# 294coder/Dif-PAN

Hardware: AMD Instinct MI355X
Metric: fused megapixels/sec at T=1000, WV3 64x64x8 tiles (higher is better)
Workload: dtype f32-class (f16x2 split); 1 GPU; WV3 pansharpening, batch 64 of 64x64x8 tiles per GPU, T=1000 DDPM p_sample, fp32; tiles_per_gpu=64, tiles_total=64, T=1000, model_evaluations=1000, sampler=ddpm, parallelism=tile-shard x1, launches_per_denoising_step=132

## Files before the change

### dif-pan_amd/csrc/ddif_dev.h

```cpp
#pragma once
#include <hip/hip_runtime.h>

#ifdef DDIF_EMU
typedef hipemu_f32x16 f32x16;
typedef hipemu_f32x4 f32x4;
#define DDIF_MFMA_32x32x2(a, b, c) hipemu_mfma_32x32x2((a), (b), (c))
#define DDIF_MFMA_16x16x4(a, b, c) hipemu_mfma_16x16x4((a), (b), (c))
static inline f32x16 ddif_mfma_bf16_emu(float4 a, float4 b, f32x16 c) {
    hipemu_u32x4 ua, ub;
    __builtin_memcpy(&ua, &a, 16);
    __builtin_memcpy(&ub, &b, 16);
    return hipemu_mfma_32x32x16_bf16(ua, ub, c);
}
#define DDIF_MFMA_32x32x16_BF16(a, b, c) ddif_mfma_bf16_emu((a), (b), (c))
static inline f32x16 ddif_mfma_f16_emu(float4 a, float4 b, f32x16 c) {
    hipemu_u32x4 ua, ub;
    __builtin_memcpy(&ua, &a, 16);
    __builtin_memcpy(&ub, &b, 16);
    return hipemu_mfma_32x32x16_f16(ua, ub, c);
}
#define DDIF_MFMA_32x32x16_F16(a, b, c) ddif_mfma_f16_emu((a), (b), (c))
#define DDIF_DYN_SMEM(name) char* name = hipemu::tctx().dyn_smem
#define DDIF_SCHED_FENCE() ((void)0)
#else
typedef float f32x16 __attribute__((ext_vector_type(16)));
typedef float f32x4 __attribute__((ext_vector_type(4)));
#define DDIF_MFMA_32x32x2(a, b, c) __builtin_amdgcn_mfma_f32_32x32x2f32((a), (b), (c), 0, 0, 0)
#define DDIF_MFMA_16x16x4(a, b, c) __builtin_amdgcn_mfma_f32_16x16x4f32((a), (b), (c), 0, 0, 0)
typedef __bf16 ddif_bf16x8 __attribute__((ext_vector_type(8)));
#define DDIF_MFMA_32x32x16_BF16(a, b, c) \
    __builtin_amdgcn_mfma_f32_32x32x16_bf16(__builtin_bit_cast(ddif_bf16x8, (a)), __builtin_bit_cast(ddif_bf16x8, (b)), (c), 0, 0, 0)
typedef _Float16 ddif_f16x8 __attribute__((ext_vector_type(8)));
#define DDIF_MFMA_32x32x16_F16(a, b, c) \
    __builtin_amdgcn_mfma_f32_32x32x16_f16(__builtin_bit_cast(ddif_f16x8, (a)), __builtin_bit_cast(ddif_f16x8, (b)), (c), 0, 0, 0)
#define DDIF_DYN_SMEM(name) extern __shared__ __attribute__((aligned(16))) char name[]
#define DDIF_SCHED_FENCE() __builtin_amdgcn_sched_barrier(0)
#endif

#define DDIF_WAVE 64
#define DDIF_GN_EPS 1e-5

#ifdef DDIF_EMU
static inline long long wall_clock64() { return 0; }
#endif

namespace ddif {

__device__ __forceinline__ float dd_exp(float x) { return expf(x); }
__device__ __forceinline__ float dd_sigmoid(float x) {
#ifdef DDIF_EMU
    return 1.0f / (1.0f + exp2f(-1.4426950408889634f * x));
#else
    return __builtin_amdgcn_rcpf(1.0f + __builtin_amdgcn_exp2f(-1.4426950408889634f * x));
#endif
}
__device__ __forceinline__ float dd_silu(float x) { return x * dd_sigmoid(x); }
__device__ __forceinline__ float dd_exp2_fast(float x) {
#ifdef DDIF_EMU
    return exp2f(x);
#else
    return __builtin_amdgcn_exp2f(x);
#endif
}
__device__ __forceinline__ float dd_rcp_fast(float x) {
#ifdef DDIF_EMU
    return 1.0f / x;
#else
    return __builtin_amdgcn_rcpf(x);
#endif
}

__device__ __forceinline__ unsigned dd_bf16_bits(float x) {
    const unsigned u = __builtin_bit_cast(unsigned, x);
    return (u + 0x7fffu + ((u >> 16) & 1u)) >> 16;
}
__device__ __forceinline__ float dd_bf16_val(unsigned b) { return __builtin_bit_cast(float, b << 16); }
__device__ __forceinline__ void dd_split3(float x, unsigned* hi, unsigned* mid, unsigned* lo) {
    const unsigned h = dd_bf16_bits(x);
    const float r1 = x - dd_bf16_val(h);
    const unsigned m = dd_bf16_bits(r1);
    const float r2 = r1 - dd_bf16_val(m);
    *hi = h;
    *mid = m;
    *lo = dd_bf16_bits(r2);
}

__device__ __forceinline__ void dd_split3_pair(float a, float b, unsigned* hi, unsigned* mid, unsigned* lo) {
#ifdef DDIF_EMU
    unsigned ha, ma, la, hb, mb, lb;
    dd_split3(a, &ha, &ma, &la);
    dd_split3(b, &hb, &mb, &lb);
    *hi = ha | (hb << 16);
    *mid = ma | (mb << 16);
    *lo = la | (lb << 16);
#else
    typedef float v2f __attribute__((ext_vector_type(2)));
    typedef __bf16 v2b __attribute__((ext_vector_type(2)));
    const v2f v = {a, b};
    const unsigned H = __builtin_bit_cast(unsigned, __builtin_convertvector(v, v2b));
    const v2f r1 = {a - __builtin_bit_cast(float, H << 16), b - __builtin_bit_cast(float, H & 0xffff0000u)};
    const unsigned M = __builtin_bit_cast(unsigned, __builtin_convertvector(r1, v2b));
    const v2f r2 = {r1.x - __builtin_bit_cast(float, M << 16), r1.y - __builtin_bit_cast(float, M & 0xffff0000u)};
    *hi = H;
    *mid = M;
    *lo = __builtin_bit_cast(unsigned, __builtin_convertvector(r2, v2b));
#endif
}

__device__ __forceinline__ unsigned dd_bf16_pair(float a, float b) {
#ifdef DDIF_EMU
    return dd_bf16_bits(a) | (dd_bf16_bits(b) << 16);
#else
    typedef float v2f __attribute__((ext_vector_type(2)));
    typedef __bf16 v2b __attribute__((ext_vector_type(2)));
    const v2f v = {a, b};
    return __builtin_bit_cast(unsigned, __builtin_convertvector(v, v2b));
#endif
}

#define DDIF_F16_ASCALE 16.0f
#define DDIF_F16_WSCALE 1024.0f
#define DDIF_F16_OSCALE (1.0f / (DDIF_F16_ASCALE * DDIF_F16_WSCALE))
#define DDIF_F16_AMAX 4094.0f
#define DDIF_F16_WMAX 63.9f
#ifdef DDIF_EMU
static inline unsigned dd_f16_bits(float x) { return hipemu_f32_to_f16(x); }
static inline float dd_f16_val(unsigned b) { return hipemu_f16_to_f32((unsigned short)b); }
#endif
__device__ __forceinline__ void dd_split2_pair(float a, float b, unsigned* hi, unsigned* lo) {
#ifdef DDIF_EMU
    const unsigned ha = dd_f16_bits(a), hb = dd_f16_bits(b);
    *hi = ha | (hb << 16);
    *lo = dd_f16_bits(a - dd_f16_val(ha)) | (dd_f16_bits(b - dd_f16_val(hb)) << 16);
#else
    typedef float v2f __attribute__((ext_vector_type(2)));
    typedef _Float16 v2h __attribute__((ext_vector_type(2)));
    const v2f v = {a, b};
    const v2h H = __builtin_convertvector(v, v2h);
    const v2f r = {a - (float)H.x, b - (float)H.y};
    *hi = __builtin_bit_cast(unsigned, H);
    *lo = __builtin_bit_cast(unsigned, __builtin_convertvector(r, v2h));
#endif
}
__device__ __forceinline__ float dd_silu_scaled(float x, float inv_s) {
#ifdef DDIF_EMU
    return x * (1.0f / fmaf(exp2f(-1.4426950408889634f * x), inv_s, inv_s));
#else
    return x * __builtin_amdgcn_rcpf(fmaf(__builtin_amdgcn_exp2f(-1.4426950408889634f * x), inv_s, inv_s));
#endif
}

__device__ __forceinline__ int dd_late(int v) {
#if !defined(DDIF_EMU) && defined(__HIP_DEVICE_COMPILE__)
    asm volatile("" : "+v"(v));
#endif
    return v;
}

template <int BYTES>
__device__ __forceinline__ void dd_touch_kernargs() {
#if !defined(DDIF_EMU) && defined(__HIP_DEVICE_COMPILE__)
    const unsigned long long ka = (unsigned long long)__builtin_amdgcn_kernarg_segment_ptr();
    static_assert(BYTES >= 4 && BYTES <= 448, "kernarg touch: up to eight loads");
    constexpr int NL = (BYTES + 63) / 64 + 1;
#define DD_KA_OFF(i) ((i) * 64 < BYTES - 4 ? (i) * 64 : BYTES - 4)
    [[maybe_unused]] unsigned d0, d1, d2, d3, d4, d5, d6, d7;
    if constexpr (NL == 2) asm volatile("s_load_dword %0, %2, %3\n\ts_load_dword %1, %2, %4\n\ts_waitcnt lgkmcnt(0)" : "=&s"(d0), "=&s"(d1) : "s"(ka), "n"(DD_KA_OFF(0)), "n"(DD_KA_OFF(1)) : "memory");
    else if constexpr (NL == 3) asm volatile("s_load_dword %0, %3, %4\n\ts_load_dword %1, %3, %5\n\ts_load_dword %2, %3, %6\n\ts_waitcnt lgkmcnt(0)" : "=&s"(d0), "=&s"(d1), "=&s"(d2) : "s"(ka), "n"(DD_KA_OFF(0)), "n"(DD_KA_OFF(1)), "n"(DD_KA_OFF(2)) : "memory");
    else if constexpr (NL == 4) asm volatile("s_load_dword %0, %4, %5\n\ts_load_dword %1, %4, %6\n\ts_load_dword %2, %4, %7\n\ts_load_dword %3, %4, %8\n\ts_waitcnt lgkmcnt(0)" : "=&s"(d0), "=&s"(d1), "=&s"(d2), "=&s"(d3) : "s"(ka), "n"(DD_KA_OFF(0)), "n"(DD_KA_OFF(1)), "n"(DD_KA_OFF(2)), "n"(DD_KA_OFF(3)) : "memory");
    else if constexpr (NL == 5) asm volatile("s_load_dword %0, %5, %6\n\ts_load_dword %1, %5, %7\n\ts_load_dword %2, %5, %8\n\ts_load_dword %3, %5, %9\n\ts_load_dword %4, %5, %10\n\ts_waitcnt lgkmcnt(0)" : "=&s"(d0), "=&s"(d1), "=&s"(d2), "=&s"(d3), "=&s"(d4) : "s"(ka), "n"(DD_KA_OFF(0)), "n"(DD_KA_OFF(1)), "n"(DD_KA_OFF(2)), "n"(DD_KA_OFF(3)), "n"(DD_KA_OFF(4)) : "memory");
    else if constexpr (NL == 6) asm volatile("s_load_dword %0, %6, %7\n\ts_load_dword %1, %6, %8\n\ts_load_dword %2, %6, %9\n\ts_load_dword %3, %6, %10\n\ts_load_dword %4, %6, %11\n\ts_load_dword %5, %6, %12\n\ts_waitcnt lgkmcnt(0)" : "=&s"(d0), "=&s"(d1), "=&s"(d2), "=&s"(d3), "=&s"(d4), "=&s"(d5) : "s"(ka), "n"(DD_KA_OFF(0)), "n"(DD_KA_OFF(1)), "n"(DD_KA_OFF(2)), "n"(DD_KA_OFF(3)), "n"(DD_KA_OFF(4)), "n"(DD_KA_OFF(5)) : "memory");
    else if constexpr (NL == 7) asm volatile("s_load_dword %0, %7, %8\n\ts_load_dword %1, %7, %9\n\ts_load_dword %2, %7, %10\n\ts_load_dword %3, %7, %11\n\ts_load_dword %4, %7, %12\n\ts_load_dword %5, %7, %13\n\ts_load_dword %6, %7, %14\n\ts_waitcnt lgkmcnt(0)" : "=&s"(d0), "=&s"(d1), "=&s"(d2), "=&s"(d3), "=&s"(d4), "=&s"(d5), "=&s"(d6) : "s"(ka), "n"(DD_KA_OFF(0)), "n"(DD_KA_OFF(1)), "n"(DD_KA_OFF(2)), "n"(DD_KA_OFF(3)), "n"(DD_KA_OFF(4)), "n"(DD_KA_OFF(5)), "n"(DD_KA_OFF(6)) : "memory");
    else if constexpr (NL == 8) asm volatile("s_load_dword %0, %8, %9\n\ts_load_dword %1, %8, %10\n\ts_load_dword %2, %8, %11\n\ts_load_dword %3, %8, %12\n\ts_load_dword %4, %8, %13\n\ts_load_dword %5, %8, %14\n\ts_load_dword %6, %8, %15\n\ts_load_dword %7, %8, %16\n\ts_waitcnt lgkmcnt(0)" : "=&s"(d0), "=&s"(d1), "=&s"(d2), "=&s"(d3), "=&s"(d4), "=&s"(d5), "=&s"(d6), "=&s"(d7) : "s"(ka), "n"(DD_KA_OFF(0)), "n"(DD_KA_OFF(1)), "n"(DD_KA_OFF(2)), "n"(DD_KA_OFF(3)), "n"(DD_KA_OFF(4)), "n"(DD_KA_OFF(5)), "n"(DD_KA_OFF(6)), "n"(DD_KA_OFF(7)) : "memory");
#undef DD_KA_OFF
#endif
}

__device__ __forceinline__ void wg_work_range(int nwork, int* w0, int* w1, int xcd = 0) {
    const unsigned g = gridDim.x, n = (unsigned)nwork;
    const unsigned b = (xcd && (g & 7u) == 0u) ? (blockIdx.x & 7u) * (g >> 3) + (blockIdx.x >> 3) : blockIdx.x;
    const unsigned q = n / g, r = n - q * g;
    *w0 = (int)(b * q + (b * r) / g);
    *w1 = (int)((b + 1) * q + ((b + 1) * r) / g);
}

__device__ __forceinline__ float wave_sum(float v) {
#pragma unroll
    for (int m = 32; m >= 1; m >>= 1) v += __shfl_xor(v, m);
    return v;
}
__device__ __forceinline__ float wave_sum_fast(float v) {
#ifdef DDIF_EMU
#pragma unroll
    for (int m = 32; m >= 1; m >>= 1) v += __shfl_xor(v, m);
    return v;
#else
    v += __builtin_bit_cast(float, __builtin_amdgcn_update_dpp(0, __builtin_bit_cast(int, v), 0xB1, 0xf, 0xf, false));
    v += __builtin_bit_cast(float, __builtin_amdgcn_update_dpp(0, __builtin_bit_cast(int, v), 0x4E, 0xf, 0xf, false));
    v += __builtin_bit_cast(float, __builtin_amdgcn_update_dpp(0, __builtin_bit_cast(int, v), 0x124, 0xf, 0xf, false));
    v += __builtin_bit_cast(float, __builtin_amdgcn_update_dpp(0, __builtin_bit_cast(int, v), 0x128, 0xf, 0xf, false));
    v += __builtin_bit_cast(float, __builtin_amdgcn_update_dpp(0, __builtin_bit_cast(int, v), 0x142, 0xa, 0xf, false));
    v += __builtin_bit_cast(float, __builtin_amdgcn_update_dpp(0, __builtin_bit_cast(int, v), 0x143, 0xc, 0xf, false));
    return v;
#endif
}
__device__ __forceinline__ double wave_sum(double v) {
#pragma unroll
    for (int m = 32; m >= 1; m >>= 1) v += __shfl_xor(v, m);
    return v;
}
__device__ __forceinline__ double wave_sum_fast_f64(double v) {
#ifdef DDIF_EMU
    return wave_sum(v);
#else
#define DDIF_DPP_ADD_F64(ctrl, rmask)                                                                              \
    {                                                                                                              \
        const unsigned long long u = __builtin_bit_cast(unsigned long long, v);                                    \
        const int lo = __builtin_amdgcn_update_dpp(0, (int)(unsigned)u, ctrl, rmask, 0xf, false);                   \
        const int hi = __builtin_amdgcn_update_dpp(0, (int)(unsigned)(u >> 32), ctrl, rmask, 0xf, false);           \
        v += __builtin_bit_cast(double, ((unsigned long long)(unsigned)hi << 32) | (unsigned long long)(unsigned)lo); \
    }
    DDIF_DPP_ADD_F64(0xB1, 0xf)
    DDIF_DPP_ADD_F64(0x4E, 0xf)
    DDIF_DPP_ADD_F64(0x124, 0xf)
    DDIF_DPP_ADD_F64(0x128, 0xf)
    DDIF_DPP_ADD_F64(0x142, 0xa)
    DDIF_DPP_ADD_F64(0x143, 0xc)
#undef DDIF_DPP_ADD_F64
    const unsigned long long u = __builtin_bit_cast(unsigned long long, v);
    const unsigned lo = (unsigned)__builtin_amdgcn_readlane((int)(unsigned)u, 63), hi = (unsigned)__builtin_amdgcn_readlane((int)(unsigned)(u >> 32), 63);
    return __builtin_bit_cast(double, ((unsigned long long)hi << 32) | lo);
#endif
}
__device__ __forceinline__ float wave_max(float v) {
#pragma unroll
    for (int m = 32; m >= 1; m >>= 1) v = fmaxf(v, __shfl_xor(v, m));
    return v;
}

struct GnRedRec { const double* cpart; float* dgamma; float* dbeta; int C, nchunk, blk0, pad; };
struct GnPartials {
    double v[2][4][2];
};
__device__ __forceinline__ void gn_load_partials(const double* st0, int np0, const double* st1, int np1, int b, GnPartials* p) {
    const int lane = threadIdx.x & 63;
#pragma unroll
    for (int k = 0; k < 4; ++k) {
        const int i = lane + 64 * k;
        const int i0 = i < np0 ? i : np0 - 1;
        p->v[0][k][0] = st0[((size_t)b * np0 + i0) * 2 + 0];
        p->v[0][k][1] = st0[((size_t)b * np0 + i0) * 2 + 1];
        if (st1 != nullptr) {
            const int i1 = i < np1 ? i : np1 - 1;
            p->v[1][k][0] = st1[((size_t)b * np1 + i1) * 2 + 0];
            p->v[1][k][1] = st1[((size_t)b * np1 + i1) * 2 + 1];
        }
    }
}
__device__ __forceinline__ void gn_reduce_partials(const GnPartials& p, const double* st0, int np0, const double* st1, int np1, int b,
                                                    double count, float* mean_out, float* rstd_out) {
    const int lane = threadIdx.x & 63;
    double s = 0.0, ss = 0.0;
#pragma unroll
    for (int k = 0; k < 4; ++k)
        if (lane + 64 * k < np0) {
            s += p.v[0][k][0];
            ss += p.v[0][k][1];
        }
    for (int i = lane + 256; i < np0; i += 64) {
        s += st0[((size_t)b * np0 + i) * 2 + 0];
        ss += st0[((size_t)b * np0 + i) * 2 + 1];
    }
    if (st1 != nullptr) {
#pragma unroll
        for (int k = 0; k < 4; ++k)
            if (lane + 64 * k < np1) {
                s += p.v[1][k][0];
                ss += p.v[1][k][1];
            }
        for (int i = lane + 256; i < np1; i += 64) {
            s += st1[((size_t)b * np1 + i) * 2 + 0];
            ss += st1[((size_t)b * np1 + i) * 2 + 1];
        }
    }
    s = wave_sum_fast_f64(s);
    ss = wave_sum_fast_f64(ss);
    const double mean = s / count;
    double var = ss / count - mean * mean;
    if (var < 0.0) var = 0.0;
    *mean_out = (float)mean;
    *rstd_out = (float)(1.0 / sqrt(var + DDIF_GN_EPS));
}
__device__ __forceinline__ void gn_finalize_wave(const double* st0, int np0, const double* st1, int np1, int b,
                                                  double count, float* mean_out, float* rstd_out) {
    GnPartials p;
    gn_load_partials(st0, np0, st1, np1, b, &p);
    gn_reduce_partials(p, st0, np0, st1, np1, b, count, mean_out, rstd_out);
}

}
```

### dif-pan_amd/csrc/kernels_lr.h

```cpp
#pragma once
#include "kernels_conv.h"

namespace ddif {

#ifndef LR_ROWPAD
#define LR_ROWPAD 1
#endif
#if defined(DDIF_EMU) || !defined(__HIP_DEVICE_COMPILE__)
#define LR_PREFETCH_FENCE() ((void)0)
#elif defined(LR_NO_FENCE)
#define LR_PREFETCH_FENCE() ((void)0)
#else
#define LR_PREFETCH_FENCE() asm volatile("" ::: "memory")
#endif
template <int KS, int MB, int PRO, bool TALL = false, bool F16 = false, bool B1 = false>
struct LrGeom {
    static constexpr int NPL = F16 ? 2 : (B1 ? 1 : 3);
    static constexpr int TH = (TALL && MB == 4) ? 16 : 8, TW = (MB == 2 || TALL) ? 8 : 16;
    static constexpr int PAD = KS / 2;
    static constexpr int IH = TH + 2 * PAD, IW = TW + 2 * PAD;
    static constexpr int PC = (MB == 4 && KS == 3) ? 64 : 128;
    static constexpr int SP = PC / 16;
    static constexpr int APIX = SP * NPL * 8 + 4;
    static constexpr int RSL = (IW * APIX / 4) % 16;
    static constexpr int RPAD = LR_ROWPAD ? (((TW == 8 ? 8 : 0) - RSL + 16) % 16) * 4 : 0;
    static constexpr int AROW = IW * APIX + RPAD;
    static constexpr int AFL = IH * AROW;
    static constexpr int RFL = 4 * MB * 4 * 64 * 4;
    static constexpr size_t smem = (size_t)((AFL > RFL ? AFL : RFL) + 16) * sizeof(float);
    static constexpr int SPW = SP / 4;
    static constexpr int TAPS = KS * KS;
    static constexpr int U = KS == 3 ? TAPS : SPW;
};

template <int KS, int MB, int PRO, int EPI, int ABL = 0, bool F16 = false, bool B1 = false, bool ROWS = false>
__global__ __launch_bounds__(256) void conv_lr_kernel(ConvArgs a) {
    constexpr bool COLST = (EPI & EPI_COLST) != 0;
    static_assert(!COLST || KS == 1, "column statistics epilogue: 1x1 convs");
    static_assert(!F16 || PRO != PRO_COLSM, "f16x2: the column-softmax prologue stays on bf16x3");
    static_assert(!(F16 && B1), "one operand format");
    using G = LrGeom<KS, MB, PRO, COLST, F16, B1>;
    constexpr int NPL = G::NPL, SLF = NPL * 8;
    constexpr int WSTEP = NPL * 1024;
    constexpr int TH = G::TH, TW = G::TW, LP = G::PAD, LH = G::IH, LW = G::IW, IW = G::IW, PC = G::PC, SP = G::SP;
    constexpr int APIX = G::APIX, AROW = G::AROW, TAPS = G::TAPS, U = G::U, SPW = G::SPW;
    constexpr bool GNP = (PRO == PRO_GN || PRO == PRO_GN_SILU);
    static_assert(PRO == PRO_NONE || PRO == PRO_GN || PRO == PRO_GN_SILU || PRO == PRO_COLSM, "prologues of the low-resolution kernel");
    constexpr bool FILM = (EPI & EPI_FILM) != 0, RES = (EPI & EPI_RES) != 0, SILU = (EPI & EPI_SILU) != 0;
    constexpr int C4 = PC / 4;
    constexpr int PSTEP = 256 / C4;
    constexpr int NIT = ROWS ? LH : (LH * LW + PSTEP - 1) / PSTEP;
    static_assert(256 % C4 == 0, "staging geometry");
    static_assert(!ROWS || (KS == 3 && PSTEP == TW && PRO != PRO_COLSM), "row staging: 3x3 convs, one pass of the threads = one image row");

    dd_touch_kernargs<sizeof(ConvArgs)>();
    DDIF_DYN_SMEM(smem);
    float* As = reinterpret_cast<float*>(smem);
    float* Red = As;
    float* Sst = As + (G::AFL > G::RFL ? G::AFL : G::RFL);

    const int tid = threadIdx.x, lane = tid & 63;
#ifdef DDIF_EMU
    const int wave = tid >> 6;
#else
    const int wave = __builtin_amdgcn_readfirstlane(tid >> 6);
#endif
    const int h = lane >> 5, j = lane & 31;
    const int tiles = a.tiles_x * a.tiles_y;
    const int nwork = a.B * tiles * a.n_ct;
    int w0, w1;
    wg_work_range(nwork, &w0, &w1, a.xcd);
    const int Ctot = a.c0 + a.c1;
#ifdef DDIF_EMU
    const int ac0 = a.c0, ac1 = a.c1;
#else
    const int ac0 = __builtin_amdgcn_readfirstlane(a.c0), ac1 = __builtin_amdgcn_readfirstlane(a.c1);
#endif
    const int NS = (Ctot + 15) / 16;
    const int NSW = a.n_chunks * (KS == 3 ? 1 : 2);
    const int NP = (NS + SP - 1) / SP;
    const int c4 = tid % C4, p0 = tid / C4;
    const int stepv = a.step_ptr ? *a.step_ptr : 0;

    int abase[MB];
#pragma unroll
    for (int mb = 0; mb < MB; ++mb) {
        const int m = mb * 32 + j;
        abase[mb] = (m / TW) * AROW + (m % TW) * APIX + 4 * h;
    }

    int gn_b = -1;
    float mean = 0.f, rstd = 1.f;
    constexpr bool RANGE = F16 && !GNP && PRO != PRO_COLSM;
    [[maybe_unused]] float r_max = 0.f;

    for (int work = w0; work < w1; ++work) {
        const int pt = work / a.n_ct, ct = work - pt * a.n_ct;
        const int bl = pt / tiles, t = pt - bl * tiles;
        const int b = a.b0 + bl;
        const int oy0 = (t / a.tiles_x) * TH, ox0 = (t % a.tiles_x) * TW;

        [[maybe_unused]] GnPartials gp;
        const bool new_b = GNP && b != gn_b;
        if (new_b) gn_load_partials(a.st0, a.np0, a.st1, a.np1, b, &gp);

        const int co = ct * 32 + 8 * wave + 4 * h;
        const bool cok_o = co < a.Cout;
        const int coc = cok_o ? co : 0;
        const float4 bq = *reinterpret_cast<const float4*>(a.bias + coc);
        [[maybe_unused]] float4 e_res[RES ? MB : 1], e_fs[FILM ? MB : 1], e_fh[FILM ? MB : 1];
        bool pok[MB];
        size_t opix[MB];
#pragma unroll
        for (int mb = 0; mb < MB; ++mb) {
            const int m = mb * 32 + j;
            const int oy = oy0 + m / TW, ox = ox0 + m % TW;
            pok[mb] = (oy < a.Hout) & (ox < a.Wout) & cok_o;
            opix[mb] = pok[mb] ? ((size_t)b * a.Hout + oy) * a.Wout + ox : 0;
            if constexpr (RES) e_res[mb] = *reinterpret_cast<const float4*>(a.res + opix[mb] * a.Cout + coc);
            if constexpr (FILM) {
                e_fs[mb] = *reinterpret_cast<const float4*>(a.film + opix[mb] * 2 * a.Cout + coc);
                e_fh[mb] = *reinterpret_cast<const float4*>(a.film + opix[mb] * 2 * a.Cout + a.Cout + coc);
            }
        }

        const char* wbase = reinterpret_cast<const char*>(a.w + (size_t)b * a.w_bstride) + ((size_t)ct * NSW * TAPS) * WSTEP + (size_t)lane * 16;
        int pf_slab = wave, pf_tap = 0;
        float4 wr[U][NPL];
        auto ring_load = [&](int slot) {
            const int s = pf_slab < NS ? pf_slab : 0;
            const char* p = wbase + ((size_t)s * TAPS + pf_tap) * WSTEP;
#pragma unroll
            for (int q = 0; q < NPL; ++q) {
                if (ABL & 1) wr[slot][q] = make_float4(1e-3f * (float)q, 2e-3f, 3e-3f, 4e-3f);
                else wr[slot][q] = *reinterpret_cast<const float4*>(p + q * 1024);
            }
            if (++pf_tap == TAPS) {
                pf_tap = 0;
                pf_slab += 4;
            }
        };
#pragma unroll
        for (int u = 0; u < U; ++u) ring_load(u);

        float4 sv[NIT];
        [[maybe_unused]] float4 mxv[PRO == PRO_COLSM ? NIT : 1], smv[PRO == PRO_COLSM ? NIT : 1];
        [[maybe_unused]] float4 gq4, bq4;
        unsigned okm = 0;
        auto stage_load = [&](int ph) {
            const int c = ph * PC + c4 * 4;
            const bool cok = c < Ctot;
            const bool s0 = !cok || c < a.c0;
            const float* src = s0 ? a.in0 + (cok ? c : 0) : a.in1 + (c - a.c0);
            const int cs = s0 ? ac0 : ac1;
            okm = 0;
            if constexpr (ROWS) {
                const float* rp = src + (((size_t)b * a.Hin + oy0) * a.Win + p0) * cs;
                const ptrdiff_t rs = (ptrdiff_t)a.Win * cs;
#pragma unroll
                for (int it = 0; it < NIT; ++it) {
                    const int iy = oy0 - LP + it;
                    if ((iy >= 0) & (iy < a.Hin)) {
                        okm |= 1u << it;
                        if (ABL & 4) sv[it] = make_float4(0.5f, 0.25f, -0.5f, 0.125f);
                        else sv[it] = *reinterpret_cast<const float4*>(rp + (ptrdiff_t)(it - LP) * rs);
                    }
                }
            } else {
#pragma unroll
            for (int it = 0; it < NIT; ++it) {
                const int pix = p0 + it * PSTEP;
                const int py = pix / LW, px = pix - py * LW;
                const int iy = oy0 - LP + py, ix = ox0 - LP + px;
                const bool ok = (pix < LH * LW) & (iy >= 0) & (iy < a.Hin) & (ix >= 0) & (ix < a.Win) & cok;
                okm |= (ok ? 1u : 0u) << it;
                const int iyc = iy < 0 ? 0 : (iy >= a.Hin ? a.Hin - 1 : iy), ixc = ix < 0 ? 0 : (ix >= a.Win ? a.Win - 1 : ix);
                const size_t sp = ((size_t)b * a.Hin + iyc) * a.Win + ixc;
                if (ABL & 4) sv[it] = make_float4(0.5f, 0.25f, -0.5f, 0.125f);
                else sv[it] = *reinterpret_cast<const float4*>(src + sp * cs);
                if constexpr (PRO == PRO_COLSM) {
                    const size_t so = ((size_t)b * a.Win + ixc) * a.c0 + ((s0 && cok) ? c : 0);
                    mxv[it] = *reinterpret_cast<const float4*>(a.cs_mx + so);
                    smv[it] = *reinterpret_cast<const float4*>(a.cs_sm + so);
                }
            }
            }
            if constexpr (GNP) {
                gq4 = *reinterpret_cast<const float4*>(a.gamma + (cok ? c : 0));
                bq4 = *reinterpret_cast<const float4*>(a.beta + (cok ? c : 0));
            }
        };
        auto stage_write = [&](int ph) {
            const int c = ph * PC + c4 * 4;
            const bool cok = c < Ctot;
            const bool colsm = (PRO == PRO_COLSM) && cok && c < a.c0;
            const int slab_l = (c4 * 4) / 16, cin_slab = (c4 * 4) % 16;
            float ga[4] = {1.f, 1.f, 1.f, 1.f}, gb[4] = {0.f, 0.f, 0.f, 0.f};
            if constexpr (GNP) {
#pragma unroll
                for (int i = 0; i < 4; ++i) {
                    ga[i] = (&gq4.x)[i] * rstd;
                    gb[i] = (&bq4.x)[i] - mean * ga[i];
                    if constexpr (F16 && PRO == PRO_GN) {
                        ga[i] *= DDIF_F16_ASCALE;
                        gb[i] *= DDIF_F16_ASCALE;
                    }
                }
            }
#pragma unroll
            for (int it = 0; it < NIT; ++it) {
                const int pix = ROWS ? it * LW + p0 + LP : p0 + it * PSTEP;
                if constexpr (ROWS) {
                    if (!((okm >> it) & 1u)) {
                        float* d = &As[it * AROW + (p0 + LP) * APIX + slab_l * SLF + cin_slab / 2];
#pragma unroll
                        for (int q = 0; q < NPL; ++q) *reinterpret_cast<uint2*>(d + 8 * q) = make_uint2(0u, 0u);
                        continue;
                    }
                }
                const bool ok = ROWS ? cok : (okm >> it) & 1u;
                float v[4];
#pragma unroll
                for (int i = 0; i < 4; ++i) {
                    float x = (&sv[it].x)[i];
                    if constexpr (GNP) {
                        x = fmaf(x, ga[i], gb[i]);
                        if constexpr (PRO == PRO_GN_SILU) x = F16 ? dd_silu_scaled(x, 1.0f / DDIF_F16_ASCALE) : dd_silu(x);
                    } else if constexpr (F16) {
                        x *= DDIF_F16_ASCALE;
                    }
                    if constexpr (PRO == PRO_COLSM) {
                        if (colsm) x = dd_exp2_fast((x - (&mxv[it].x)[i]) * 1.4426950408889634f) * dd_rcp_fast((&smv[it].x)[i]);
                    }
                    v[i] = ok ? x : 0.f;
                }
                if constexpr (RANGE) r_max = fmaxf(fmaxf(r_max, fmaxf(fabsf(v[0]), fabsf(v[1]))), fmaxf(fabsf(v[2]), fabsf(v[3])));
                if (ROWS || pix < LH * LW) {
                    float* d = ROWS ? &As[it * AROW + (p0 + LP) * APIX + slab_l * SLF + cin_slab / 2] : &As[(pix / LW) * AROW + (pix % LW) * APIX + slab_l * SLF + cin_slab / 2];
                    if constexpr (B1) {
                        *reinterpret_cast<uint2*>(d) = make_uint2(dd_bf16_pair(v[0], v[1]), dd_bf16_pair(v[2], v[3]));
                    } else if constexpr (F16) {
                        unsigned h01, l01, h23, l23;
                        dd_split2_pair(v[0], v[1], &h01, &l01);
                        dd_split2_pair(v[2], v[3], &h23, &l23);
                        *reinterpret_cast<uint2*>(d) = make_uint2(h01, h23);
                        *reinterpret_cast<uint2*>(d + 8) = make_uint2(l01, l23);
                    } else {
                        unsigned h01, m01, l01, h23, m23, l23;
                        dd_split3_pair(v[0], v[1], &h01, &m01, &l01);
                        dd_split3_pair(v[2], v[3], &h23, &m23, &l23);
                        *reinterpret_cast<uint2*>(d) = make_uint2(h01, h23);
                        *reinterpret_cast<uint2*>(d + 8) = make_uint2(m01, m23);
                        *reinterpret_cast<uint2*>(d + 16) = make_uint2(l01, l23);
                    }
                }
            }
        };
        stage_load(0);
        if constexpr (ROWS) {
            constexpr int Q = (APIX - 4) / 4;
            for (int i = tid; i < LH * 2 * Q; i += 256) {
                const int r = i / (2 * Q), e = i - r * (2 * Q);
                *reinterpret_cast<float4*>(&As[r * AROW + (e >= Q ? (LW - 1) * APIX + (e - Q) * 4 : e * 4)]) = make_float4(0.f, 0.f, 0.f, 0.f);
            }
        }
        const float4 tq = *reinterpret_cast<const float4*>(a.tbias + (size_t)dd_late(stepv) * a.tb_rowstride + (size_t)b * a.tbias_stride + coc);

        if (new_b) {
            gn_reduce_partials(gp, a.st0, a.np0, a.st1, a.np1, b, (double)Ctot * a.Hin * a.Win, &mean, &rstd);
            gn_b = b;
        }
        f32x16 acc[MB];
#pragma unroll
        for (int mb = 0; mb < MB; ++mb)
#pragma unroll
            for (int r = 0; r < 16; ++r) acc[mb][r] = 0.f;

        for (int ph = 0; ph < NP; ++ph) {
            if (ph > 0) __syncthreads();
            stage_write(ph);
            if (ph + 1 < NP) stage_load(ph + 1);
            __syncthreads();
            const int s_end = (ph + 1) * SP < NS ? (ph + 1) * SP : NS;
            float4 xa[2][MB][NPL];
            auto a_load = [&](int buf, int sl, int tap) {
                const int aoff = (tap / KS) * AROW + (tap % KS) * APIX + sl * SLF;
#pragma unroll
                for (int q = 0; q < NPL; ++q)
#pragma unroll
                    for (int mb = 0; mb < MB; ++mb) xa[buf][mb][q] = *reinterpret_cast<const float4*>(&As[abase[mb] + aoff + q * 8]);
            };
#pragma unroll
            for (int k = 0; k < SPW; ++k) {
                const int sl = wave + 4 * k;
                if (ph * SP + sl < s_end) {
                    a_load(0, sl, 0);
#pragma unroll
                    for (int tap = 0; tap < TAPS; ++tap) {
                        constexpr int UU = U;
                        const int u = (k * TAPS + tap) % UU;
                        const int cur = tap & 1;
                        if (tap + 1 < TAPS) a_load(cur ^ 1, sl, tap + 1);
                        LR_PREFETCH_FENCE();
                        if (ABL & 2) {
#pragma unroll
                            for (int mb = 0; mb < MB; ++mb) acc[mb][0] += wr[u][0].x * xa[cur][mb][0].x + wr[u][NPL / 2].y * xa[cur][mb][NPL / 2].y + wr[u][NPL - 1].z * xa[cur][mb][NPL - 1].z;
                        } else if constexpr (B1) {
#pragma unroll
                            for (int mb = 0; mb < MB; ++mb) acc[mb] = DDIF_MFMA_32x32x16_BF16(wr[u][0], xa[cur][mb][0], acc[mb]);
                        } else if constexpr (F16) {
#pragma unroll
                            for (int mb = 0; mb < MB; ++mb) acc[mb] = DDIF_MFMA_32x32x16_F16(wr[u][NPL - 1], xa[cur][mb][0], acc[mb]);
#pragma unroll
                            for (int mb = 0; mb < MB; ++mb) acc[mb] = DDIF_MFMA_32x32x16_F16(wr[u][0], xa[cur][mb][NPL - 1], acc[mb]);
#pragma unroll
                            for (int mb = 0; mb < MB; ++mb) acc[mb] = DDIF_MFMA_32x32x16_F16(wr[u][0], xa[cur][mb][0], acc[mb]);
                        } else if constexpr (NPL == 3) {
#pragma unroll
                            for (int mb = 0; mb < MB; ++mb) acc[mb] = DDIF_MFMA_32x32x16_BF16(wr[u][2], xa[cur][mb][0], acc[mb]);
#pragma unroll
                            for (int mb = 0; mb < MB; ++mb) acc[mb] = DDIF_MFMA_32x32x16_BF16(wr[u][0], xa[cur][mb][2], acc[mb]);
#pragma unroll
                            for (int mb = 0; mb < MB; ++mb) acc[mb] = DDIF_MFMA_32x32x16_BF16(wr[u][1], xa[cur][mb][1], acc[mb]);
#pragma unroll
                            for (int mb = 0; mb < MB; ++mb) acc[mb] = DDIF_MFMA_32x32x16_BF16(wr[u][1], xa[cur][mb][0], acc[mb]);
#pragma unroll
                            for (int mb = 0; mb < MB; ++mb) acc[mb] = DDIF_MFMA_32x32x16_BF16(wr[u][0], xa[cur][mb][1], acc[mb]);
#pragma unroll
                            for (int mb = 0; mb < MB; ++mb) acc[mb] = DDIF_MFMA_32x32x16_BF16(wr[u][0], xa[cur][mb][0], acc[mb]);
                        }
                        if (pf_slab < NS) ring_load(u);
                    }
                }
            }
        }
        __syncthreads();
#pragma unroll
        for (int mb = 0; mb < MB; ++mb)
#pragma unroll
            for (int g = 0; g < 4; ++g)
                *reinterpret_cast<float4*>(&Red[(((wave * MB + mb) * 4 + g) * 64 + lane) * 4]) =
                    make_float4(acc[mb][4 * g + 0], acc[mb][4 * g + 1], acc[mb][4 * g + 2], acc[mb][4 * g + 3]);
        __syncthreads();
        float s1 = 0.f, s2 = 0.f;
        [[maybe_unused]] float colv[COLST ? MB : 1][4];
#pragma unroll
        for (int mb = 0; mb < MB; ++mb) {
            float4 pp[4];
#pragma unroll
            for (int w = 0; w < 4; ++w) pp[w] = *reinterpret_cast<const float4*>(&Red[(((w * MB + mb) * 4 + wave) * 64 + lane) * 4]);
            float v[4];
#pragma unroll
            for (int i = 0; i < 4; ++i) {
                float x = ((&pp[0].x)[i] + (&pp[1].x)[i]) + ((&pp[2].x)[i] + (&pp[3].x)[i]);
                x = F16 ? fmaf(x, DDIF_F16_OSCALE, (&bq.x)[i] + (&tq.x)[i]) : x + ((&bq.x)[i] + (&tq.x)[i]);
                if constexpr (FILM) x = x * (1.f + (&e_fs[mb].x)[i]) + (&e_fh[mb].x)[i];
                if constexpr (SILU) x = dd_silu(x);
                if constexpr (RES) x += (&e_res[mb].x)[i];
                v[i] = x;
            }
            if constexpr (COLST) {
#pragma unroll
                for (int i = 0; i < 4; ++i) colv[mb][i] = pok[mb] ? v[i] : -INFINITY;
            }
            if (pok[mb]) {
                if (!(ABL & 8) || v[0] == 12345.678f) *reinterpret_cast<float4*>(a.out + opix[mb] * a.Cout + co) = make_float4(v[0], v[1], v[2], v[3]);
                s1 += (v[0] + v[1]) + (v[2] + v[3]);
                s2 += (v[0] * v[0] + v[1] * v[1]) + (v[2] * v[2] + v[3] * v[3]);
            }
        }
        if constexpr (COLST) {
            float cm[4], cs[4];
#pragma unroll
            for (int i = 0; i < 4; ++i) {
                float m = colv[0][i];
#pragma unroll
                for (int mb = 1; mb < MB; ++mb) m = fmaxf(m, colv[mb][i]);
                m = fmaxf(m, __shfl_xor(m, 8));
                m = fmaxf(m, __shfl_xor(m, 16));
                float e = 0.f;
#pragma unroll
                for (int mb = 0; mb < MB; ++mb) e += dd_exp(colv[mb][i] - m);
                e += __shfl_xor(e, 8);
                e += __shfl_xor(e, 16);
                cm[i] = m;
                cs[i] = e;
            }
            const int ox = ox0 + (j & 7);
            if (j < 8 && ox < a.Wout && cok_o) {
                const size_t so = ((size_t)b * a.Wout + ox) * a.Cout + co;
                *reinterpret_cast<float4*>(a.cso_mx + so) = make_float4(cm[0], cm[1], cm[2], cm[3]);
                *reinterpret_cast<float4*>(a.cso_sm + so) = make_float4(cs[0], cs[1], cs[2], cs[3]);
            }
        }
        if (a.st_out) {
            const float t1 = wave_sum_fast(s1), t2 = wave_sum_fast(s2);
            if (lane == 63) {
                Sst[wave * 2 + 0] = t1;
                Sst[wave * 2 + 1] = t2;
            }
        }
        __syncthreads();
        if (a.st_out && tid == 0) {
            const size_t pi = ((size_t)b * (tiles * a.n_ct) + (size_t)t * a.n_ct + ct) * 2;
            a.st_out[pi + 0] = ((double)Sst[0] + (double)Sst[2]) + ((double)Sst[4] + (double)Sst[6]);
            a.st_out[pi + 1] = ((double)Sst[1] + (double)Sst[3]) + ((double)Sst[5] + (double)Sst[7]);
        }
    }
    if constexpr (RANGE) {
        if (a.range_flag && !(r_max < 65520.f)) *a.range_flag = 1;
    }
}

}
```

Before: 0.07849 MP/s.

## Cut address arithmetic and register pressure in LR conv kernel

```diff
diff --git a/dif-pan_amd/csrc/ddif_dev.h b/dif-pan_amd/csrc/ddif_dev.h
--- a/dif-pan_amd/csrc/ddif_dev.h
+++ b/dif-pan_amd/csrc/ddif_dev.h
@@ -291,6 +291,51 @@
     *mean_out = (float)mean;
     *rstd_out = (float)(1.0 / sqrt(var + DDIF_GN_EPS));
 }
+#ifndef DDIF_GN_SMALL_NP
+#define DDIF_GN_SMALL_NP 64
+#endif
+static_assert(DDIF_GN_SMALL_NP == 64 || DDIF_GN_SMALL_NP == 0, "one pair per lane is fetched ahead, or none is used");
+__device__ __forceinline__ void gn_load_partials_few(const double* st0, int np0, const double* st1, int np1, int b, GnPartials* p) {
+    const int lane = threadIdx.x & 63;
+    const unsigned i0 = (unsigned)(b * np0 + (lane < np0 ? lane : np0 - 1)) * 2u;
+    p->v[0][0][0] = st0[i0 + 0];
+    p->v[0][0][1] = st0[i0 + 1];
+    if (st1 != nullptr) {
+        const unsigned i1 = (unsigned)(b * np1 + (lane < np1 ? lane : np1 - 1)) * 2u;
+        p->v[1][0][0] = st1[i1 + 0];
+        p->v[1][0][1] = st1[i1 + 1];
+    }
+}
+__device__ __forceinline__ void gn_reduce_partials_few(const GnPartials& p, const double* st0, int np0, const double* st1, int np1, int b,
+                                                        double count, float* mean_out, float* rstd_out) {
+    const int lane = threadIdx.x & 63;
+    double s = 0.0, ss = 0.0;
+    if (DDIF_GN_SMALL_NP > 0 && lane < np0) {
+        s += p.v[0][0][0];
+        ss += p.v[0][0][1];
+    }
+    for (int i = lane + DDIF_GN_SMALL_NP; i < np0; i += 64) {
+        s += st0[((size_t)b * np0 + i) * 2 + 0];
+        ss += st0[((size_t)b * np0 + i) * 2 + 1];
+    }
+    if (st1 != nullptr) {
+        if (DDIF_GN_SMALL_NP > 0 && lane < np1) {
+            s += p.v[1][0][0];
+            ss += p.v[1][0][1];
+        }
+        for (int i = lane + DDIF_GN_SMALL_NP; i < np1; i += 64) {
+            s += st1[((size_t)b * np1 + i) * 2 + 0];
+            ss += st1[((size_t)b * np1 + i) * 2 + 1];
+        }
+    }
+    s = wave_sum_fast_f64(s);
+    ss = wave_sum_fast_f64(ss);
+    const double mean = s / count;
+    double var = ss / count - mean * mean;
+    if (var < 0.0) var = 0.0;
+    *mean_out = (float)mean;
+    *rstd_out = (float)(1.0 / sqrt(var + DDIF_GN_EPS));
+}
 __device__ __forceinline__ void gn_finalize_wave(const double* st0, int np0, const double* st1, int np1, int b,
                                                   double count, float* mean_out, float* rstd_out) {
     GnPartials p;
diff --git a/dif-pan_amd/csrc/kernels_lr.h b/dif-pan_amd/csrc/kernels_lr.h
--- a/dif-pan_amd/csrc/kernels_lr.h
+++ b/dif-pan_amd/csrc/kernels_lr.h
@@ -82,27 +82,27 @@
     const int c4 = tid % C4, p0 = tid / C4;
     const int stepv = a.step_ptr ? *a.step_ptr : 0;
 
-    int abase[MB];
-#pragma unroll
-    for (int mb = 0; mb < MB; ++mb) {
-        const int m = mb * 32 + j;
-        abase[mb] = (m / TW) * AROW + (m % TW) * APIX + 4 * h;
-    }
-
     int gn_b = -1;
     float mean = 0.f, rstd = 1.f;
     constexpr bool RANGE = F16 && !GNP && PRO != PRO_COLSM;
     [[maybe_unused]] float r_max = 0.f;
 
+    int ct, t, bl, ty, tx;
+    {
+        const unsigned pt = (unsigned)w0 / (unsigned)a.n_ct;
+        ct = w0 - (int)pt * a.n_ct;
+        bl = (int)(pt / (unsigned)tiles);
+        t = (int)pt - bl * tiles;
+        ty = ROWS ? t : (int)((unsigned)t / (unsigned)a.tiles_x);
+        tx = ROWS ? 0 : t - ty * a.tiles_x;
+    }
     for (int work = w0; work < w1; ++work) {
-        const int pt = work / a.n_ct, ct = work - pt * a.n_ct;
-        const int bl = pt / tiles, t = pt - bl * tiles;
         const int b = a.b0 + bl;
-        const int oy0 = (t / a.tiles_x) * TH, ox0 = (t % a.tiles_x) * TW;
+        const int oy0 = ty * TH, ox0 = ROWS ? 0 : tx * TW;
 
         [[maybe_unused]] GnPartials gp;
         const bool new_b = GNP && b != gn_b;
-        if (new_b) gn_load_partials(a.st0, a.np0, a.st1, a.np1, b, &gp);
+        if (new_b) gn_load_partials_few(a.st0, a.np0, a.st1, a.np1, b, &gp);
 
         const int co = ct * 32 + 8 * wave + 4 * h;
         const bool cok_o = co < a.Cout;
@@ -110,39 +110,46 @@
         const float4 bq = *reinterpret_cast<const float4*>(a.bias + coc);
         [[maybe_unused]] float4 e_res[RES ? MB : 1], e_fs[FILM ? MB : 1], e_fh[FILM ? MB : 1];
         bool pok[MB];
-        size_t opix[MB];
+        unsigned opix[MB];
 #pragma unroll
         for (int mb = 0; mb < MB; ++mb) {
             const int m = mb * 32 + j;
             const int oy = oy0 + m / TW, ox = ox0 + m % TW;
-            pok[mb] = (oy < a.Hout) & (ox < a.Wout) & cok_o;
-            opix[mb] = pok[mb] ? ((size_t)b * a.Hout + oy) * a.Wout + ox : 0;
-            if constexpr (RES) e_res[mb] = *reinterpret_cast<const float4*>(a.res + opix[mb] * a.Cout + coc);
+            pok[mb] = (oy < a.Hout) & (ROWS || ox < a.Wout) & cok_o;
+            opix[mb] = pok[mb] ? (unsigned)((b * a.Hout + oy) * a.Wout + ox) : 0u;
+            if constexpr (RES) e_res[mb] = *reinterpret_cast<const float4*>(reinterpret_cast<const char*>(a.res) + (opix[mb] * (unsigned)a.Cout + (unsigned)coc) * 4u);
             if constexpr (FILM) {
-                e_fs[mb] = *reinterpret_cast<const float4*>(a.film + opix[mb] * 2 * a.Cout + coc);
-                e_fh[mb] = *reinterpret_cast<const float4*>(a.film + opix[mb] * 2 * a.Cout + a.Cout + coc);
-            }
-        }
-
-        const char* wbase = reinterpret_cast<const char*>(a.w + (size_t)b * a.w_bstride) + ((size_t)ct * NSW * TAPS) * WSTEP + (size_t)lane * 16;
+                const unsigned fo = (opix[mb] * 2u * (unsigned)a.Cout + (unsigned)coc) * 4u;
+                e_fs[mb] = *reinterpret_cast<const float4*>(reinterpret_cast<const char*>(a.film) + fo);
+                e_fh[mb] = *reinterpret_cast<const float4*>(reinterpret_cast<const char*>(a.film) + (fo + (unsigned)a.Cout * 4u));
+            }
+        }
+
+        const char* wbase = reinterpret_cast<const char*>(a.w + (size_t)b * a.w_bstride) + ((size_t)ct * NSW * TAPS) * WSTEP;
+        const char* wp = wbase + (unsigned)(wave * TAPS) * (unsigned)WSTEP;
+        const unsigned wlane = (unsigned)lane * 16u;
         int pf_slab = wave, pf_tap = 0;
         float4 wr[U][NPL];
-        auto ring_load = [&](int slot) {
-            const int s = pf_slab < NS ? pf_slab : 0;
-            const char* p = wbase + ((size_t)s * TAPS + pf_tap) * WSTEP;
+        const char* wfill = wbase;
+        auto ring_load = [&](int slot, bool fill) {
+            if (fill) wfill = pf_tap == 0 ? (pf_slab < NS ? wp : wbase) : wfill + WSTEP;
+            const char* p = fill ? wfill : wp;
 #pragma unroll
             for (int q = 0; q < NPL; ++q) {
                 if (ABL & 1) wr[slot][q] = make_float4(1e-3f * (float)q, 2e-3f, 3e-3f, 4e-3f);
-                else wr[slot][q] = *reinterpret_cast<const float4*>(p + q * 1024);
-            }
+                else wr[slot][q] = *reinterpret_cast<const float4*>(p + (wlane + (unsigned)(q * 1024)));
+            }
+            wp += WSTEP;
             if (++pf_tap == TAPS) {
                 pf_tap = 0;
                 pf_slab += 4;
+                wp += 3 * TAPS * WSTEP;
             }
         };
 #pragma unroll
-        for (int u = 0; u < U; ++u) ring_load(u);
-
+        for (int u = 0; u < U; ++u) ring_load(u, true);
+
+        int c4_l = c4, p0_l = p0, lane_l = lane;
         float4 sv[NIT];
         [[maybe_unused]] float4 mxv[PRO == PRO_COLSM ? NIT : 1], smv[PRO == PRO_COLSM ? NIT : 1];
         [[maybe_unused]] float4 gq4, bq4;
@@ -155,15 +162,15 @@
             const int cs = s0 ? ac0 : ac1;
             okm = 0;
             if constexpr (ROWS) {
-                const float* rp = src + (((size_t)b * a.Hin + oy0) * a.Win + p0) * cs;
-                const ptrdiff_t rs = (ptrdiff_t)a.Win * cs;
+                const int rs = a.Win * cs;
+                const float* rp = src + (unsigned)(((b * a.Hin + oy0) * a.Win + p0) * cs);
 #pragma unroll
                 for (int it = 0; it < NIT; ++it) {
                     const int iy = oy0 - LP + it;
                     if ((iy >= 0) & (iy < a.Hin)) {
                         okm |= 1u << it;
                         if (ABL & 4) sv[it] = make_float4(0.5f, 0.25f, -0.5f, 0.125f);
-                        else sv[it] = *reinterpret_cast<const float4*>(rp + (ptrdiff_t)(it - LP) * rs);
+                        else sv[it] = *reinterpret_cast<const float4*>(rp + (it - LP) * rs);
                     }
                 }
             } else {
@@ -172,14 +179,14 @@
                 const int pix = p0 + it * PSTEP;
                 const int py = pix / LW, px = pix - py * LW;
                 const int iy = oy0 - LP + py, ix = ox0 - LP + px;
-                const bool ok = (pix < LH * LW) & (iy >= 0) & (iy < a.Hin) & (ix >= 0) & (ix < a.Win) & cok;
+                const bool ok = (pix < LH * LW) & (LP == 0 || iy >= 0) & (iy < a.Hin) & (LP == 0 || ix >= 0) & (ix < a.Win) & cok;
                 okm |= (ok ? 1u : 0u) << it;
-                const int iyc = iy < 0 ? 0 : (iy >= a.Hin ? a.Hin - 1 : iy), ixc = ix < 0 ? 0 : (ix >= a.Win ? a.Win - 1 : ix);
-                const size_t sp = ((size_t)b * a.Hin + iyc) * a.Win + ixc;
+                const int iyc = (LP > 0 && iy < 0) ? 0 : (iy >= a.Hin ? a.Hin - 1 : iy), ixc = (LP > 0 && ix < 0) ? 0 : (ix >= a.Win ? a.Win - 1 : ix);
+                const unsigned sp = (unsigned)((b * a.Hin + iyc) * a.Win + ixc);
                 if (ABL & 4) sv[it] = make_float4(0.5f, 0.25f, -0.5f, 0.125f);
-                else sv[it] = *reinterpret_cast<const float4*>(src + sp * cs);
+                else sv[it] = *reinterpret_cast<const float4*>(reinterpret_cast<const char*>(src) + sp * (unsigned)cs * 4u);
                 if constexpr (PRO == PRO_COLSM) {
-                    const size_t so = ((size_t)b * a.Win + ixc) * a.c0 + ((s0 && cok) ? c : 0);
+                    const size_t so = (size_t)(b * a.Win + ixc) * a.c0 + ((s0 && cok) ? c : 0);
                     mxv[it] = *reinterpret_cast<const float4*>(a.cs_mx + so);
                     smv[it] = *reinterpret_cast<const float4*>(a.cs_sm + so);
                 }
@@ -191,10 +198,10 @@
             }
         };
         auto stage_write = [&](int ph) {
-            const int c = ph * PC + c4 * 4;
+            const int c = ph * PC + c4_l * 4;
             const bool cok = c < Ctot;
             const bool colsm = (PRO == PRO_COLSM) && cok && c < a.c0;
-            const int slab_l = (c4 * 4) / 16, cin_slab = (c4 * 4) % 16;
+            const int slab_l = (c4_l * 4) / 16, cin_slab = (c4_l * 4) % 16;
             float ga[4] = {1.f, 1.f, 1.f, 1.f}, gb[4] = {0.f, 0.f, 0.f, 0.f};
             if constexpr (GNP) {
 #pragma unroll
@@ -209,10 +216,10 @@
             }
 #pragma unroll
             for (int it = 0; it < NIT; ++it) {
-                const int pix = ROWS ? it * LW + p0 + LP : p0 + it * PSTEP;
+                const int pix = ROWS ? it * LW + p0_l + LP : p0_l + it * PSTEP;
                 if constexpr (ROWS) {
                     if (!((okm >> it) & 1u)) {
-                        float* d = &As[it * AROW + (p0 + LP) * APIX + slab_l * SLF + cin_slab / 2];
+                        float* d = &As[it * AROW + (p0_l + LP) * APIX + slab_l * SLF + cin_slab / 2];
 #pragma unroll
                         for (int q = 0; q < NPL; ++q) *reinterpret_cast<uint2*>(d + 8 * q) = make_uint2(0u, 0u);
                         continue;
@@ -236,7 +243,7 @@
                 }
                 if constexpr (RANGE) r_max = fmaxf(fmaxf(r_max, fmaxf(fabsf(v[0]), fabsf(v[1]))), fmaxf(fabsf(v[2]), fabsf(v[3])));
                 if (ROWS || pix < LH * LW) {
-                    float* d = ROWS ? &As[it * AROW + (p0 + LP) * APIX + slab_l * SLF + cin_slab / 2] : &As[(pix / LW) * AROW + (pix % LW) * APIX + slab_l * SLF + cin_slab / 2];
+                    float* d = ROWS ? &As[it * AROW + (p0_l + LP) * APIX + slab_l * SLF + cin_slab / 2] : &As[(pix / LW) * AROW + (pix % LW) * APIX + slab_l * SLF + cin_slab / 2];
                     if constexpr (B1) {
                         *reinterpret_cast<uint2*>(d) = make_uint2(dd_bf16_pair(v[0], v[1]), dd_bf16_pair(v[2], v[3]));
                     } else if constexpr (F16) {
@@ -266,8 +273,19 @@
         }
         const float4 tq = *reinterpret_cast<const float4*>(a.tbias + (size_t)dd_late(stepv) * a.tb_rowstride + (size_t)b * a.tbias_stride + coc);
 
+        const int tid_l = ROWS ? dd_late(tid) : tid;
+        lane_l = tid_l & 63;
+        c4_l = tid_l % C4;
+        p0_l = tid_l / C4;
+        int abase[MB];
+#pragma unroll
+        for (int mb = 0; mb < MB; ++mb) {
+            const int m = mb * 32 + (lane_l & 31);
+            abase[mb] = (m / TW) * AROW + (m % TW) * APIX + 4 * (lane_l >> 5);
+        }
+
         if (new_b) {
-            gn_reduce_partials(gp, a.st0, a.np0, a.st1, a.np1, b, (double)Ctot * a.Hin * a.Win, &mean, &rstd);
+            gn_reduce_partials_few(gp, a.st0, a.np0, a.st1, a.np1, b, (double)dd_late(Ctot) * a.Hin * a.Win, &mean, &rstd);
             gn_b = b;
         }
         f32x16 acc[MB];
@@ -329,7 +347,7 @@
 #pragma unroll
                             for (int mb = 0; mb < MB; ++mb) acc[mb] = DDIF_MFMA_32x32x16_BF16(wr[u][0], xa[cur][mb][0], acc[mb]);
                         }
-                        if (pf_slab < NS) ring_load(u);
+                        if (pf_slab < NS) ring_load(u, false);
                     }
                 }
             }
@@ -339,7 +357,7 @@
         for (int mb = 0; mb < MB; ++mb)
 #pragma unroll
             for (int g = 0; g < 4; ++g)
-                *reinterpret_cast<float4*>(&Red[(((wave * MB + mb) * 4 + g) * 64 + lane) * 4]) =
+                *reinterpret_cast<float4*>(&Red[(((wave * MB + mb) * 4 + g) * 64 + lane_l) * 4]) =
                     make_float4(acc[mb][4 * g + 0], acc[mb][4 * g + 1], acc[mb][4 * g + 2], acc[mb][4 * g + 3]);
         __syncthreads();
         float s1 = 0.f, s2 = 0.f;
@@ -348,7 +366,7 @@
         for (int mb = 0; mb < MB; ++mb) {
             float4 pp[4];
 #pragma unroll
-            for (int w = 0; w < 4; ++w) pp[w] = *reinterpret_cast<const float4*>(&Red[(((w * MB + mb) * 4 + wave) * 64 + lane) * 4]);
+            for (int w = 0; w < 4; ++w) pp[w] = *reinterpret_cast<const float4*>(&Red[(((w * MB + mb) * 4 + wave) * 64 + lane_l) * 4]);
             float v[4];
 #pragma unroll
             for (int i = 0; i < 4; ++i) {
@@ -364,7 +382,7 @@
                 for (int i = 0; i < 4; ++i) colv[mb][i] = pok[mb] ? v[i] : -INFINITY;
             }
             if (pok[mb]) {
-                if (!(ABL & 8) || v[0] == 12345.678f) *reinterpret_cast<float4*>(a.out + opix[mb] * a.Cout + co) = make_float4(v[0], v[1], v[2], v[3]);
+                if (!(ABL & 8) || v[0] == 12345.678f) *reinterpret_cast<float4*>(reinterpret_cast<char*>(a.out) + (opix[mb] * (unsigned)a.Cout + (unsigned)co) * 4u) = make_float4(v[0], v[1], v[2], v[3]);
                 s1 += (v[0] + v[1]) + (v[2] + v[3]);
                 s2 += (v[0] * v[0] + v[1] * v[1]) + (v[2] * v[2] + v[3] * v[3]);
             }
@@ -406,6 +424,21 @@
             a.st_out[pi + 0] = ((double)Sst[0] + (double)Sst[2]) + ((double)Sst[4] + (double)Sst[6]);
             a.st_out[pi + 1] = ((double)Sst[1] + (double)Sst[3]) + ((double)Sst[5] + (double)Sst[7]);
         }
+        if (++ct == a.n_ct) {
+            ct = 0;
+            ++t;
+            if (ROWS) ++ty;
+            else if (++tx == a.tiles_x) {
+                tx = 0;
+                ++ty;
+            }
+            if (t == tiles) {
+                t = 0;
+                ty = 0;
+                tx = 0;
+                ++bl;
+            }
+        }
     }
     if constexpr (RANGE) {
         if (a.range_flag && !(r_max < 65520.f)) *a.range_flag = 1;
```

Result: no change. 0.07926 MP/s (median of 6 runs) (+1.0%).
